# m4rch1n0/vqvae

Hardware: AMD Instinct MI355X
Metric: latents/sec through geodesic kNN+APSP+K-medoids (higher is better)
Workload: dtype f64-exact(u32 fixed point)

## Files before the change

include/geo_hip.h:

```cpp
#ifndef GEO_HIP_H
#define GEO_HIP_H

#include <stddef.h>
#include <stdint.h>

#ifdef __cplusplus
extern "C" {
#endif

#define GEO_OK 0
#define GEO_E_ARG (-1)
#define GEO_E_WORKSPACE (-2)
#define GEO_E_HIP (-3)
#define GEO_E_NOCONV (-4)

int geo_version(void);
const char *geo_last_error(void);

int geo_set_option(const char *name, int32_t value);

size_t geo_sssp_workspace_bytes(int32_t n, int64_t nnz, int32_t n_sources);

int geo_sssp_multi(const int32_t *indptr, const int32_t *indices, const float *weights,
                   int32_t n, int64_t nnz, const int32_t *sources, int32_t n_sources,
// ... 95 lines not shown
size_t geo_jvp_edges_workspace_bytes(const geo_decoder_desc *dec, int64_t n_nodes, int64_t n_edges, int32_t batch_size);
int geo_decoder_jvp_edges(const geo_decoder_desc *dec, const float *z, int64_t n_nodes,
                          const int32_t *src, const int32_t *dst, int64_t n_edges, int32_t batch_size,
                          float *len_out, void *ws, size_t ws_bytes, void *stream);

#define GEO_JVP_FRONT_VALU 0
#define GEO_JVP_FRONT_MFMA 1
#define GEO_JVP_MID_PIPE 0
#define GEO_JVP_MID_PIPE_DEDUP 1
#define GEO_JVP_MID_ALL 2
#define GEO_JVP_MID_ALL_TANGENT 3
#define GEO_JVP_MID_CHUNK 4
#define GEO_JVP_BACK_MFMA 0
#define GEO_JVP_BACK_PER_NODE 1
#define GEO_JVP_BACK_DEDUP 2
#define GEO_JVP_BACK_VALU 3
#define GEO_JVP_PLAN_FRONT(p) ((p) & 3)
#define GEO_JVP_PLAN_DMAX(p) (16 << (((p) >> 2) & 3))
#define GEO_JVP_PLAN_MID(p) (((p) >> 4) & 15)
#define GEO_JVP_PLAN_BACK(p) (((p) >> 8) & 15)
#define GEO_JVP_PER_NODE 0x1000
#define GEO_JVP_NODE_JACOBIAN 0x2000
#define GEO_JVP_DEDUP 0x4000
#define GEO_JVP_PLAN_PASSES(p) ((p) >> 16)
int geo_jvp_plan(const geo_decoder_desc *dec, int64_t n_nodes, int64_t n_edges, int32_t batch_size, int32_t graph_edges,
                 size_t ws_bytes);

int geo_decoder_jvp_pairs(const geo_decoder_desc *dec, const float *z_start, const float *z_end,
                          int64_t n_edges, int32_t batch_size, float *len_out,
                          void *ws, size_t ws_bytes, void *stream);

typedef struct geo_vanilla_decoder_desc {
    int32_t latent_dim;
    int32_t c1, c2;
    int32_t out_channels;
    int32_t out_size;
    const float *At;
    const float *c;
    const float *w2p;
    const float *scale2;
    const float *shift2;
    const float *w3p;
    const float *b3;
} geo_vanilla_decoder_desc;

size_t geo_vanilla_jvp_workspace_bytes(const geo_vanilla_decoder_desc *dec, int64_t n_edges);
// ... 87 lines not shown
```

vqvae_amd/_lib.py:

```python
import ctypes
import os

import torch

_HERE = os.path.dirname(os.path.abspath(__file__))
LIB_PATH = os.path.join(_HERE, "libgeo_hip.so")

c_p = ctypes.c_void_p
i32, i64, sz = ctypes.c_int32, ctypes.c_int64, ctypes.c_size_t


class DecoderDesc(ctypes.Structure):
    _fields_ = ([(n, i32) for n in ("latent_dim", "c0", "c1", "c2", "out_channels", "out_size", "norm",
                                    "bn_train", "groups1", "groups2")]
                + [("eps", ctypes.c_float)]
                + [(n, c_p) for n in ("w_in", "b_in", "w1", "b1", "g1", "be1", "rm1", "rv1",
                                      "w2", "b2", "g2", "be2", "rm2", "rv2", "w3", "b3")]
                + [("update_running", i32), ("momentum", ctypes.c_float)])


class VanillaDecoderDesc(ctypes.Structure):
    _fields_ = ([(n, i32) for n in ("latent_dim", "c1", "c2", "out_channels", "out_size")]
                + [(n, c_p) for n in ("At", "c", "w2p", "scale2", "shift2", "w3p", "b3")])

# ... 65 lines not shown
    "geo_feature_gram": (ctypes.c_int, [c_p, i64, i32, i64, c_p, c_p, c_p, c_p, sz, c_p]),
    "geo_feature_project": (ctypes.c_int, [c_p, i64, i32, i64, c_p, c_p, c_p, i32, c_p, c_p]),
    "geo_vq_workspace_bytes": (sz, [i64, i32, i32]),
    "geo_vq_forward": (ctypes.c_int, [c_p, i32, i32, i32, i32, c_p, c_p, c_p, i32, i32, ctypes.c_double, ctypes.c_double,
                                      ctypes.c_double, c_p, c_p, c_p, c_p, c_p, c_p, c_p, sz, c_p]),
    "geo_vq_backward": (ctypes.c_int, [c_p, c_p, ctypes.c_double, c_p, i32, c_p, i64, c_p, c_p]),
    "geo_vae_elbo_workspace_bytes": (sz, [i64, i64, i64]),
    "geo_vae_elbo_forward": (ctypes.c_int, [c_p, c_p, c_p, c_p, i64, i64, i64, i32, i32, ctypes.c_double, ctypes.c_double,
                                            ctypes.c_double, i32, c_p, c_p, sz, c_p]),
    "geo_vae_elbo_backward": (ctypes.c_int, [c_p, c_p, c_p, c_p, c_p, c_p, i64, i64, i64, i32, i32, ctypes.c_double,
                                             ctypes.c_double, ctypes.c_double, i32, c_p, c_p, c_p, c_p]),
    "geo_batch_assemble": (ctypes.c_int, [c_p, i64, i32, i32, i32, c_p, i32, c_p, c_p, i32, c_p, c_p, c_p, c_p]),
}

EXPORTS = tuple(_SIGNATURES)

JVP_FRONT = ("valu", "mfma")
JVP_MID = ("pipe", "pipe_dedup", "all", "all_tangent", "chunk")
JVP_BACK = ("mfma", "per_node", "dedup", "valu")


def decode_jvp_plan(code: int) -> dict:
    assert code >= 0, code
    return {"front": JVP_FRONT[code & 3], "dmax": 16 << ((code >> 2) & 3), "mid": JVP_MID[(code >> 4) & 15],
            "back": JVP_BACK[(code >> 8) & 15], "per_node": bool(code & 0x1000), "node_jacobian": bool(code & 0x2000),
            "dedup": bool(code & 0x4000), "passes": code >> 16}
_lib = None


class GeoHipError(RuntimeError):
    pass


def load() -> ctypes.CDLL:
    global _lib
    if _lib is None:
        if not os.path.exists(LIB_PATH):
            raise GeoHipError(
                f"{LIB_PATH} is missing: build it with `make -C vqvae_amd/csrc` "
                "(the geodesic-codebook path has no CPU fallback)")
        L = ctypes.CDLL(LIB_PATH)
        for name, (res, args) in _SIGNATURES.items():
            fn = getattr(L, name)
            fn.restype, fn.argtypes = res, args
        _lib = L
    return _lib


def check(status: int, what: str) -> None:
# ... 3 lines not shown
```

vqvae_amd/csrc/common.hip:

```cpp
#include "geo_common.h"

#include <cstdlib>
#include <cstring>

namespace geo {

namespace {
struct OptionName { const char *name, *env; int Options::*field; };
const OptionName kOptionNames[] = {
    {"sssp_sb", "GEO_SSSP_SB", &Options::sssp_sb},
    {"sssp_act", "GEO_SSSP_ACT", &Options::sssp_act},
    {"sssp_sparse_div", "GEO_SSSP_SPARSE_DIV", &Options::sssp_sparse_div},
    {"sssp_map_div", "GEO_SSSP_MAP_DIV", &Options::sssp_map_div},
    {"sssp_group", "GEO_SSSP_GROUP", &Options::sssp_group},
    {"sssp_grouped_cap", "GEO_SSSP_GROUPED_CAP", &Options::sssp_grouped_cap},
    {"sssp_trace", "GEO_SSSP_TRACE", &Options::sssp_trace},
    {"sssp_u32", "GEO_SSSP_U32", &Options::sssp_u32},
    {"sssp_push", "GEO_SSSP_PUSH", &Options::sssp_push},
    {"sssp_order", "GEO_SSSP_ORDER", &Options::sssp_order},
    {"sssp_delta", "GEO_SSSP_DELTA", &Options::sssp_delta},
    {"sssp_push_blocks", "GEO_SSSP_PUSH_BLOCKS", &Options::sssp_push_blocks},
    {"knn_filter", "GEO_KNN_FILTER", &Options::knn_filter},
    {"kpp_grid", "GEO_KPP_GRID", &Options::kpp_grid},
    {"kpp_profile", "GEO_KPP_PROFILE", &Options::kpp_profile},
    {"jvp_mid", "GEO_JVP_MID", &Options::jvp_mid},
    {"jvp_back_valu", "GEO_JVP_BACK_VALU", &Options::jvp_back_valu},
    {"jvp_front_valu", "GEO_JVP_FRONT_VALU", &Options::jvp_front_valu},
    {"jvp_per_node", "GEO_JVP_PER_NODE", &Options::jvp_per_node},
    {"jvp_node_jacobian", "GEO_JVP_NODE_JACOBIAN", &Options::jvp_node_jacobian},
    {"jvp_start_dedup", "GEO_JVP_START_DEDUP", &Options::jvp_start_dedup},
};
Options from_environment() {
    Options o;
    for (const OptionName &e : kOptionNames) {
        const char *v = getenv(e.env);
        if (!v) continue;
        if (e.field == &Options::jvp_mid) o.jvp_mid = v[0] == 'c' ? 2 : (v[0] == 'a' ? 3 : atoi(v));
        else o.*(e.field) = atoi(v);
    }
    return o;
}
}

Options &options() {
    static Options o = from_environment();
    return o;
}

static thread_local char g_err[512] = "";

void set_error(const char *fmt, ...) {
    va_list ap;
    va_start(ap, fmt);
// ... 87 lines not shown
    int rc = scan_rec(sums, offs, t, ar, s);
    if (rc != GEO_OK) return rc;
    scan_add_kernel<<<dim3((unsigned)t), dim3(SCAN_THREADS), 0, s>>>(out, offs, n, t);
    GEO_LAUNCH_CHECK();
    return GEO_OK;
}

int exclusive_scan_i32(const int32_t *in, int32_t *out, int64_t n, void *tmp, size_t tmp_bytes,
                       int64_t *total_host, hipStream_t stream) {
    Arena ar(tmp, tmp_bytes);
    int rc = scan_rec(in, out, n, ar, stream);
    if (rc != GEO_OK) return rc;
    if (total_host) {
        int32_t tot = 0;
        GEO_HIP_CHECK(hipMemcpyAsync(&tot, out + n, sizeof(int32_t), hipMemcpyDeviceToHost, stream));
        GEO_HIP_CHECK(hipStreamSynchronize(stream));
        *total_host = tot;
    }
    return GEO_OK;
}

}

extern "C" int geo_version(void) { return 104; }
extern "C" const char *geo_last_error(void) { return geo::g_err; }

extern "C" int geo_set_option(const char *name, int32_t value) {
    if (name)
        for (const geo::OptionName &e : geo::kOptionNames)
            if (strcmp(name, e.name) == 0) {
                geo::options().*(e.field) = value;
                return GEO_OK;
            }
    geo::set_error("geo_set_option: unknown option '%s'", name ? name : "(null)");
    return GEO_E_ARG;
}
```

vqvae_amd/csrc/geo_common.h:

```cpp
#pragma once
#include <hip/hip_runtime.h>

#include <cstdarg>
#include <cstdint>
#include <cstdio>

#include "geo_hip.h"

namespace geo {

void set_error(const char *fmt, ...);

#define GEO_HIP_CHECK(expr)                                                                      \
    do {                                                                                         \
        hipError_t _e = (expr);                                                                  \
        if (_e != hipSuccess) {                                                                  \
            geo::set_error("%s failed: %s (%s:%d)", #expr, hipGetErrorString(_e), __FILE__, __LINE__); \
            return GEO_E_HIP;                                                                    \
        }                                                                                        \
    } while (0)

#define GEO_REQUIRE(cond, ...)              \
    do {                                    \
        if (!(cond)) {                      \
            geo::set_error(__VA_ARGS__);    \
            return GEO_E_ARG;               \
        }                                   \
    } while (0)

#define GEO_LAUNCH_CHECK() GEO_HIP_CHECK(hipGetLastError())

struct Options {
    int sssp_sb = -1, sssp_act = 1, sssp_sparse_div = -1, sssp_map_div = -1, sssp_group = 1, sssp_grouped_cap = 256,
        sssp_trace = 0, sssp_u32 = 1, sssp_push = 1 ,
        sssp_delta = 8 , sssp_order = 0 , sssp_push_blocks = 64, knn_filter = 1, kpp_grid = 256, kpp_profile = 0, jvp_mid = 0 ,
        jvp_back_valu = 0, jvp_front_valu = 0, jvp_per_node = 1 ,
        jvp_node_jacobian = 1 ,
        jvp_start_dedup = 1 ;
};
Options &options();

static inline size_t align_up(size_t x, size_t a = 256) { return (x + a - 1) / a * a; }

struct Arena {
    char *base;
    size_t size, off;
    Arena(void *p, size_t n) : base(static_cast<char *>(p)), size(n), off(0) {}
    template <typename T>
    T *take(size_t count) {
        size_t bytes = align_up(count * sizeof(T));
        if (off + bytes > size) return nullptr;
        T *r = reinterpret_cast<T *>(base + off);
        off += bytes;
        return r;
    }
};

size_t scan_tmp_bytes(int64_t n);
int exclusive_scan_i32(const int32_t *in, int32_t *out, int64_t n, void *tmp, size_t tmp_bytes,
                       int64_t *total_host, hipStream_t stream);

// ... 9 lines not shown
```

vqvae_amd/csrc/jvp.hip:

```cpp
#include "geo_common.h"

#include <cmath>
#include <cstdlib>
#include <type_traits>
#include <vector>

namespace {

constexpr int TS = 32;
constexpr int NC = 128;
constexpr int MAX_BLOCKS = 4;
constexpr int FRONT_MAX_N1 = 1024;
constexpr int BACK_TS = 8;

typedef float f32x16 __attribute__((ext_vector_type(16)));
typedef __bf16 bf16x8 __attribute__((ext_vector_type(8)));
typedef unsigned short u16x8 __attribute__((ext_vector_type(8)));

struct Shape {
    int d, c0, c1, c2, co, s_out, pad3, p_out;
    int n1, n2;
    int opix_per_chunk, n_chunks;
};

// ... 119 lines not shown
            }
#pragma unroll
            for (int u = 0; u < 2; ++u) {
                const float x = u ? x2.y : x2.x, t = u ? t2.y : t2.x;
                pre[(slot0 + s + u) * n1 + n] = x;
                tpre[(slot0 + s + u) * n1 + n] = t;
                if (valid_s[s + u]) {
                    sx += x; sxx += (double)x * x; st += t; sxt += (double)x * t;
                }
            }
        }
        if (want_stats) { ps[n][0] = sx; ps[n][1] = sxx; ps[n][2] = st; ps[n][3] = sxt; }
    }
    if (want_stats) {
        __syncthreads();
        const int c1 = n1 / 4;
        for (int c = threadIdx.x; c < c1; c += 256) {
            double a0 = 0, a1 = 0, a2 = 0, a3 = 0;
#pragma unroll
            for (int px = 0; px < 4; ++px) { a0 += ps[px * c1 + c][0]; a1 += ps[px * c1 + c][1]; a2 += ps[px * c1 + c][2]; a3 += ps[px * c1 + c][3]; }
            double *p = partial + ((size_t)tile * c1 + c) * 4;
            p[0] = a0; p[1] = a1; p[2] = a2; p[3] = a3;
        }
    }
}

template <int DMAX>
__global__ __launch_bounds__(256) void front_mfma_kernel(const float *__restrict__ z, const int32_t *__restrict__ src,
                                                        const int32_t *__restrict__ dst, const float *__restrict__ z_start,
                                                        const float *__restrict__ z_end, int64_t e_base, int64_t n_edges,
                                                        int batch, int tiles_per_group, int d, int n1,
                                                        const float *__restrict__ M01, const float *__restrict__ b01,
                                                        float *__restrict__ pre, float *__restrict__ tpre,
                                                        double *__restrict__ partial, int want_stats) {
    __shared__ float zp[TS][DMAX + 1];
    __shared__ float dz[TS][DMAX + 1];
    __shared__ int valid_s[TS];
    __shared__ double ps[FRONT_MAX_N1][4];
    const int tile = blockIdx.x;
    const int group = tile / tiles_per_group, tg = tile % tiles_per_group;
    const int chunk = group >> 1, side = group & 1;
    for (int i = threadIdx.x; i < TS * DMAX; i += 256) {
        const int s = i / DMAX, k = i % DMAX;
        const int within = tg * TS + s;
        const int64_t e = e_base + (int64_t)chunk * batch + within;
        float a = 0.f, b = 0.f;
// ... 836 lines not shown
            tile = next;
        }
        epilogue(tile - (int)gridDim.x);
    }
#undef GEO_STAGE_FULL
#undef GEO_PIPE_SEP
#undef GEO_PB
#undef GEO_PIPE_PIXEL
}

__global__ __launch_bounds__(256) void start_runs_kernel(const int32_t *__restrict__ src, int64_t e_base, int64_t n_edges, int batch,
                                                        int slots_per_group, int32_t *__restrict__ row_map, int32_t *__restrict__ rep,
                                                        int32_t *__restrict__ n_compact) {
    __shared__ int wsum[4];
    __shared__ int carry_s;
    const int chunk = blockIdx.x;
    const size_t g0 = (size_t)chunk * 2 * slots_per_group;
    const int lane = threadIdx.x & 63, wave = threadIdx.x >> 6;
    int carry = 0;
    for (int w0 = 0; w0 < slots_per_group; w0 += 256) {
        const int within = w0 + (int)threadIdx.x;
        const int64_t e = e_base + (int64_t)chunk * batch + within;
        const bool valid = within < slots_per_group && within < batch && e < n_edges;
        const bool head = valid && (within == 0 || src[e] != src[e - 1]);
        const unsigned long long m = __ballot(head);
        const int below = __popcll(m & ((1ull << lane) - 1ull));
        if (lane == 0) wsum[wave] = __popcll(m);
        __syncthreads();
        int before = carry, total = carry;
        for (int w = 0; w < 4; ++w) { if (w < wave) before += wsum[w]; total += wsum[w]; }
        const int k = before + below + (head ? 1 : 0) - 1;
        if (within < slots_per_group) {
            row_map[g0 + within] = (int32_t)(g0 + (valid ? k : 0));
            if (head) rep[g0 + k] = (int32_t)(g0 + within);
        }
        carry = total;
        __syncthreads();
    }
    if (threadIdx.x == 0) { carry_s = carry; n_compact[chunk] = carry; }
    __syncthreads();
    const int cnt = carry_s, padded = (cnt + TS - 1) / TS * TS;
    for (int k = cnt + (int)threadIdx.x; k < padded; k += 256) rep[g0 + k] = (int32_t)g0;
}

template <bool TT>
__global__ __launch_bounds__(512, 2) void mid_start_kernel(const float *__restrict__ pre1, const float *__restrict__ tpre1,
                                                          const NormConst *__restrict__ consts1, int tiles_per_group,
                                                          const unsigned short *__restrict__ B3, const float *__restrict__ b2,
                                                          float *__restrict__ pre2, float *__restrict__ tpre2,
                                                          double *__restrict__ partial2, const int32_t *__restrict__ row_map,
                                                          const int32_t *__restrict__ rep, const int32_t *__restrict__ n_compact,
                                                          int64_t e_base, int64_t n_edges, int batch) {
    constexpr int C1 = 128, LDK = C1 + 8, KS = C1 / 16, NL = 4, c2 = 64, n1 = 4 * C1, n2 = 16 * c2;
    typedef float f32x2 __attribute__((ext_vector_type(2)));
    __shared__ __attribute__((aligned(16))) unsigned short A3[2][3][2][TS][LDK];
    const int chunk = blockIdx.y, group = 2 * chunk;
    const int ncomp = TT ? 0 : n_compact[chunk];
    auto run = [&](int item) {
    const int lt0 = 2 * item;
    const bool live1 = TT ? lt0 + 1 < tiles_per_group : (lt0 + 1) * TS < ncomp;
    const int tile0 = group * tiles_per_group + lt0, tile1 = live1 ? tile0 + 1 : tile0;
    const int lane = threadIdx.x & 63, wave = __builtin_amdgcn_readfirstlane((int)(threadIdx.x >> 6));
    const int wq = wave & 3, wg = wave >> 2;
    const int r = lane & 31, h = lane >> 5;
    f32x16 accp[NL], acct[NL];
#pragma unroll
    for (int lc = 0; lc < NL; ++lc)
#pragma unroll
        for (int i = 0; i < 16; ++i) { accp[lc][i] = 0.f; acct[lc][i] = 0.f; }

    const int k0p = 2 * lane, s0p = 4 * wave;
    const NormConst *kp = consts1 + (size_t)group * C1 + k0p;
    const NormConst kA = kp[0], kB = kp[1];
    size_t xrow[2][4];
#pragma unroll
    for (int i = 0; i < 4; ++i) {
        const size_t s0 = (size_t)tile0 * TS + s0p + i, s1 = (size_t)tile1 * TS + s0p + i;
        xrow[0][i] = TT ? s0 : (size_t)__builtin_amdgcn_readfirstlane(rep[s0]);
        xrow[1][i] = TT ? s1 : (size_t)__builtin_amdgcn_readfirstlane(rep[s1]);
    }
    f32x2 rx[2][4], rt[2][4];
    auto fetch = [&](int nx) {
#pragma unroll
        for (int hh = 0; hh < 2; ++hh)
#pragma unroll
            for (int i = 0; i < 4; ++i) {
                const size_t off = xrow[hh][i] * n1 + (size_t)MidGeom::pix(nx) * C1 + k0p;
                rx[hh][i] = *reinterpret_cast<const f32x2 *>(pre1 + off);
                if (TT) rt[hh][i] = *reinterpret_cast<const f32x2 *>(tpre1 + off);
            }
    };
    fetch(0);
    auto stage_px = [&](int buf, int nx) {
#pragma unroll
        for (int hh = 0; hh < 2; ++hh)
#pragma unroll
            for (int i = 0; i < 4; ++i) {
                float a0, t0, a1, t1;
                norm_relu(kA, rx[hh][i].x, TT ? rt[hh][i].x : 0.f, &a0, &t0);
                norm_relu(kB, rx[hh][i].y, TT ? rt[hh][i].y : 0.f, &a1, &t1);
                unsigned w[3];
                if (TT) split3_pair(t0, t1, w[0], w[1], w[2]);
                else split3_pair(a0, a1, w[0], w[1], w[2]);
#pragma unroll
                for (int part = 0; part < 3; ++part) *reinterpret_cast<unsigned *>(&A3[buf][part][hh][s0p + i][k0p]) = w[part];
            }
        if (nx < 4) {
            fetch(nx);
            __builtin_amdgcn_sched_group_barrier(0x020, TT ? 16 : 8, 0);
// ... 495 lines not shown
    b += geo::align_up((size_t)16 * s.c2 * 192 * 3 * 2);
    b += 2 * geo::align_up(slots * s.n1 * 4) + 2 * geo::align_up(slots * s.n2 * 4);
    b += geo::align_up(tiles * s.n1 * 4 * 8) + geo::align_up(tiles * s.n2 * 4 * 8);
    b += geo::align_up((groups + 1) * s.c1 * sizeof(NormConst)) + geo::align_up((groups + 1) * s.c2 * sizeof(NormConst));
    b += geo::align_up((groups + 1) * (size_t)(s.c1 > s.c2 ? s.c1 : s.c2) * sizeof(float2));
    b += geo::align_up(slots * 4) * 2;
    if (dc->norm == 2) b += 2 * geo::align_up(slots * 32 * sizeof(float4));
    p->bytes = b + 4096;
    return true;
}

enum { BACK_NODE_PRIMAL = 15 };

struct Route {
    int status = GEO_OK;
    char error[192] = "";
    Plan pl = {};
    int64_t run_edges = 0, passes = 0;
    bool batch_stats = false, track = false, group_norm = false;
    int front = GEO_JVP_FRONT_VALU, dmax = 16;
    int mid = GEO_JVP_MID_CHUNK, back = GEO_JVP_BACK_VALU;
    int back_nt = 0;
    int parts2 = 16;
    bool per_node = false, node_jacobian = false, dedup = false;
    size_t back_lds = 0;
    size_t jac_np = 0, jac_extra_bytes = 0;
    size_t bytes = 0;
};

bool route_error(Route *r, int status, const char *fmt, ...) {
    va_list ap;
    va_start(ap, fmt);
    vsnprintf(r->error, sizeof(r->error), fmt, ap);
    va_end(ap);
    r->status = status;
    return false;
}

bool make_route(const geo_decoder_desc *dc, const geo::Options &o, bool graph_edges, int64_t n_nodes, int64_t n_edges, int batch,
                const size_t *ws_bytes, Route *r) {
    *r = Route{};
    if (!dc) return route_error(r, GEO_E_ARG, "geo_decoder_jvp: null pointer");
    if (batch <= 0) return route_error(r, GEO_E_ARG, "geo_decoder_jvp: batch_size must be positive");
    Plan base;
    if (n_edges < 0 || n_nodes < 0 || !make_plan(dc, n_edges, batch, &base))
        return route_error(r, GEO_E_ARG, "geo_decoder_jvp: unsupported decoder (out_size %d, c2=%d must divide %d)", dc->out_size,
                           dc->c2, NC);
// ... 15 lines not shown
    Plan jpl;
    const int64_t n_pseudo = (n_nodes + 1) / 2 * s.d;
    size_t jac_bytes = 0;
    if (per_node_kernels && n_nodes > 0 && n_edges > 0 && s.d <= 16 && o.jvp_node_jacobian != 0 &&
        (o.jvp_node_jacobian != 1 || 4 * n_edges >= 3 * n_nodes * s.d) && n_pseudo < (int64_t)1 << 31 &&
        make_plan(dc, n_pseudo, batch, &jpl) && node_slots <= jpl.pass_slots()) {
        r->jac_np = (size_t)r->back_nt * 32;
        r->jac_extra_bytes = 2 * geo::align_up((size_t)n_pseudo * 4) + geo::align_up((size_t)n_nodes * s.d * r->jac_np * 4);
        jac_bytes = r->jac_extra_bytes + jpl.bytes + node_bytes(s, n_nodes);
    }
    r->bytes = jac_bytes > per_edge_end_bytes ? jac_bytes : per_edge_end_bytes;
    const size_t ws = ws_bytes ? *ws_bytes : r->bytes;
    r->node_jacobian = jac_bytes && ws >= jac_bytes;
    r->pl = r->node_jacobian ? jpl : base;
    r->run_edges = r->node_jacobian ? n_pseudo : n_edges;
    const int64_t chunks = (r->run_edges + batch - 1) / batch;
    r->passes = (chunks + r->pl.chunks_per_pass - 1) / r->pl.chunks_per_pass;
    const size_t run_ws = ws - (r->node_jacobian ? r->jac_extra_bytes : 0);
    r->per_node = per_node_kernels && node_slots && node_slots <= r->pl.pass_slots() &&
                  run_ws >= r->pl.bytes + node_bytes(s, n_nodes);
    const size_t slots = r->pl.pass_slots(), tiles = slots / TS, groups = (size_t)r->pl.chunks_per_pass * 2;
    r->dedup = r->batch_stats && graph_edges && mid_pipe && back_mfma && o.jvp_start_dedup != 0 &&
               (2 * slots + groups) * 4 <= tiles * s.n1 * 4 * 8 && (size_t)r->back_nt * 32 <= (size_t)s.n1;

    r->mid = r->per_node ? GEO_JVP_MID_ALL_TANGENT
           : mid_pipe    ? (r->dedup ? GEO_JVP_MID_PIPE_DEDUP : GEO_JVP_MID_PIPE)
           : mid_all     ? GEO_JVP_MID_ALL
                         : GEO_JVP_MID_CHUNK;
    r->parts2 = mid_pipe && !r->per_node ? 4 : (mid_all ? 1 : 16);
    r->back = r->dedup ? GEO_JVP_BACK_DEDUP : r->per_node ? GEO_JVP_BACK_PER_NODE : back_mfma ? GEO_JVP_BACK_MFMA : GEO_JVP_BACK_VALU;
    r->back_lds = ((size_t)2 * BACK_TS * 16 * (s.c2 + 4) + (size_t)16 * s.co * (s.c2 + 4) + (size_t)BACK_TS * s.p_out) * 4;

    if (!(s.d >= 1 && s.d <= 64)) return route_error(r, GEO_E_ARG, "geo_decoder_jvp: latent_dim %d not in [1,64]", s.d);
    if (!(s.c1 == 128 || s.c1 == 64 || s.c1 == 32))
        return route_error(r, GEO_E_ARG, "geo_decoder_jvp: dec_channels[1]=%d not in {32,64,128}", s.c1);
    if (!(dc->norm >= 0 && dc->norm <= 2)) return route_error(r, GEO_E_ARG, "geo_decoder_jvp: unknown norm code %d", dc->norm);
    if (s.c2 % 16 != 0) return route_error(r, GEO_E_ARG, "geo_decoder_jvp: dec_channels[2]=%d must be a multiple of 16", s.c2);
    if (r->back_lds > 160 * 1024)
        return route_error(r, GEO_E_ARG, "geo_decoder_jvp: decoder too wide for the back kernel (%zu B LDS)", r->back_lds);
    if (run_ws < r->pl.bytes) return route_error(r, GEO_E_WORKSPACE, "geo_decoder_jvp: workspace %zu < %zu", run_ws, r->pl.bytes);
    if (r->group_norm && !(dc->groups1 == 32 && dc->groups2 == 32 && s.c2 == 64 && back_mfma && mid_all))
        return route_error(r, GEO_E_ARG,
                           "geo_decoder_jvp: GroupNorm needs 32 groups per layer and dec_channels[2] == 64 (got %d/%d groups, c2=%d)",
                           dc->groups1, dc->groups2, s.c2);
    return true;
}

int encode_route(const Route &r) {
    const int64_t passes = r.passes < 0x7fff ? r.passes : 0x7fff;
    return r.front | (r.dmax == 16 ? 0 : (r.dmax == 32 ? 1 : 2)) << 2 | r.mid << 4 | r.back << 8 |
           (r.per_node ? GEO_JVP_PER_NODE : 0) | (r.node_jacobian ? GEO_JVP_NODE_JACOBIAN : 0) | (r.dedup ? GEO_JVP_DEDUP : 0) |
           (int)passes << 16;
}

struct Buffers {
    float *M01, *b01, *B2p, *W3p, *pre1, *tpre1, *pre2, *tpre2, *norms;
    unsigned short *B3, *W3b;
    double *part1, *part2; NormConst *k1, *k2;
    float2 *stats;
    int32_t *slot_valid;
    float4 *gs1, *gs2;
    float *pre2_node, *sg_node;
    int32_t *row_map, *rep, *n_compact;
    float *sg_compact, *jac;
    ChunkTable tab;
};

struct Pass {
    int mid, back;
    int64_t tiles, e_base, n_edges;
    int tiles_per_group, batch, unit_d, stat;
    const float *z, *z_start, *z_end;
    const int32_t *src, *dst;
    float *mid_pre2;
    const float *back_pre2;
    int64_t slots() const { return tiles * TS; }
    int64_t groups() const { return tiles / tiles_per_group; }
};

template <int... Vs, class F>
void pick_int(int v, F &&f) { ((v == Vs ? (void)f(std::integral_constant<int, Vs>{}) : (void)0), ...); }
template <class F>
void pick_bool(bool v, F &&f) { if (v) f(std::true_type{}); else f(std::false_type{}); }

int cu_count(int *n) {
    static int n_cu = 0;
    if (n_cu == 0) {
        int devid = 0, cus = 0;
        GEO_HIP_CHECK(hipGetDevice(&devid));
        GEO_HIP_CHECK(hipDeviceGetAttribute(&cus, hipDeviceAttributeMultiprocessorCount, devid));
        n_cu = cus > 0 ? cus : 256;
    }
    *n = n_cu;
    return GEO_OK;
}

int launch_front(const Route &r, const Pass &p, const Buffers &b, hipStream_t stream) {
    const Shape &s = r.pl.sh;
    if (r.front == GEO_JVP_FRONT_MFMA)
        pick_int<32, 64>(r.dmax, [&](auto dm) {
            front_mfma_kernel<decltype(dm)::value><<<(unsigned)p.tiles, 256, 0, stream>>>(
                p.z, p.src, p.dst, p.z_start, p.z_end, p.e_base, p.n_edges, p.batch, p.tiles_per_group, s.d, s.n1, b.M01, b.b01,
                b.pre1, b.tpre1, b.part1, p.stat);
        });
    else
        pick_int<16, 32, 64>(r.dmax, [&](auto dm) {
            front_kernel<decltype(dm)::value><<<(unsigned)p.tiles, 256, 0, stream>>>(
                p.z, p.src, p.dst, p.z_start, p.z_end, p.e_base, p.n_edges, p.batch, p.tiles_per_group, s.d, s.n1, b.M01, b.b01,
                b.pre1, b.tpre1, b.part1, p.stat, p.unit_d);
        });
    GEO_LAUNCH_CHECK();
    return GEO_OK;
}

int launch_stats(const Route &r, const geo_decoder_desc *dc, int layer, const Pass &p, const Buffers &b, hipStream_t stream) {
    const Shape &s = r.pl.sh;
    const bool l1 = layer == 1;
    const int C = l1 ? s.c1 : s.c2, npx = l1 ? 4 : 16;
    if (p.stat) {
        finalize_batch_kernel<<<geo::grid_for(p.groups() * C, 256), 256, 0, stream>>>(
            l1 ? b.part1 : b.part2, p.tiles_per_group, l1 ? 1 : r.parts2, npx, C, p.e_base, p.n_edges, p.batch, l1 ? dc->g1 : dc->g2,
            l1 ? dc->be1 : dc->be2, dc->eps, l1 ? b.k1 : b.k2, (int)p.groups(), r.track ? b.stats : nullptr);
// ... 2 lines not shown
                b.stats, (int)p.groups(), C, dc->momentum, const_cast<float *>(l1 ? dc->rm1 : dc->rm2),
                const_cast<float *>(l1 ? dc->rv1 : dc->rv2));
        GEO_LAUNCH_CHECK();
    }
    if (r.group_norm) {
        const int32_t *prim_row = nullptr;
        if (!l1 && p.back == GEO_JVP_BACK_PER_NODE) {
            slot_node_kernel<<<geo::grid_for(p.slots(), 256), 256, 0, stream>>>(p.src, p.dst, p.e_base, p.n_edges, p.batch,
                                                                                p.tiles_per_group, p.slots(), b.slot_valid);
            prim_row = b.slot_valid;
        }
        group_stats_kernel<<<geo::grid_for(p.slots() * 32, 256), 256, 0, stream>>>(
            l1 ? b.pre1 : p.back_pre2, l1 ? b.tpre1 : b.tpre2, p.slots(), npx, C, 32, dc->eps, l1 ? b.gs1 : b.gs2, prim_row);
        GEO_LAUNCH_CHECK();
    }
    return GEO_OK;
}

int launch_mid(const Route &r, const geo_decoder_desc *dc, const Pass &p, const Buffers &b, hipStream_t stream) {
    const Shape &s = r.pl.sh;
    if (p.mid == GEO_JVP_MID_PIPE || p.mid == GEO_JVP_MID_PIPE_DEDUP) {
        const bool dedup = p.mid == GEO_JVP_MID_PIPE_DEDUP;
        const int64_t chunks = p.groups() / 2;
        if (dedup) {
            start_runs_kernel<<<(unsigned)chunks, 256, 0, stream>>>(p.src, p.e_base, p.n_edges, p.batch, p.tiles_per_group * TS,
                                                                    b.row_map, b.rep, b.n_compact);
            GEO_LAUNCH_CHECK();
        }
        int n_cu = 0;
        if (const int rc = cu_count(&n_cu)) return rc;
        const int64_t pipe_tiles = dedup ? p.tiles / 2 : p.tiles;
        const unsigned grid = (unsigned)std::min<int64_t>(pipe_tiles, n_cu);
        pick_bool(dedup, [&](auto end_only) {
            mid_pipe_kernel<decltype(end_only)::value><<<grid, 512, 0, stream>>>(
                b.pre1, b.tpre1, b.k1, p.stat, p.tiles_per_group, (int)pipe_tiles, s.c2, b.B3, dc->b2, p.mid_pre2, b.tpre2, b.part2,
                p.stat, p.e_base, p.n_edges, p.batch);
        });
        GEO_LAUNCH_CHECK();
        if (dedup) {
            mid_start_kernel<false><<<dim3(1, (unsigned)chunks), 512, 0, stream>>>(
                b.pre1, b.tpre1, b.k1, p.tiles_per_group, b.B3, dc->b2, p.mid_pre2, b.tpre2, b.part2, b.row_map, b.rep, b.n_compact,
                p.e_base, p.n_edges, p.batch);
            GEO_LAUNCH_CHECK();
            mid_start_kernel<true><<<dim3((unsigned)((p.tiles_per_group + 1) / 2), (unsigned)chunks), 512, 0, stream>>>(
                b.pre1, b.tpre1, b.k1, p.tiles_per_group, b.B3, dc->b2, p.mid_pre2, b.tpre2, b.part2, b.row_map, b.rep, b.n_compact,
                p.e_base, p.n_edges, p.batch);
            GEO_LAUNCH_CHECK();
        }
    } else if (p.mid == GEO_JVP_MID_ALL || p.mid == GEO_JVP_MID_ALL_TANGENT) {
        pick_int<128, 64, 32>(s.c1, [&](auto c1) {
            pick_bool(r.group_norm, [&](auto gn) {
                pick_bool(p.mid == GEO_JVP_MID_ALL_TANGENT, [&](auto tangent_only) {
                    mid_all_kernel<decltype(c1)::value, decltype(gn)::value, decltype(tangent_only)::value>
                        <<<(unsigned)p.tiles, 512, 0, stream>>>(b.pre1, b.tpre1, b.k1, p.stat, p.tiles_per_group, s.c2, b.B3, dc->b2,
                                                                p.mid_pre2, b.tpre2, b.part2, p.stat, b.slot_valid, b.gs1, p.e_base,
                                                                p.n_edges, p.batch);
                });
            });
        });
        GEO_LAUNCH_CHECK();
    } else {
        pick_int<128, 64, 32>(s.c1, [&](auto c1) {
            mid_bf16_kernel<decltype(c1)::value><<<dim3((unsigned)p.tiles, (unsigned)s.n_chunks), 256, 0, stream>>>(
                b.pre1, b.tpre1, b.k1, p.stat, p.tiles_per_group, b.tab, s.opix_per_chunk, s.c2, b.B3, dc->b2, p.mid_pre2, b.tpre2,
                b.part2, p.stat, b.slot_valid);
        });
        GEO_LAUNCH_CHECK();
    }
    return GEO_OK;
// ... 21 lines not shown
                p.back_pre2, b.tpre2, b.k2, 1, p.tiles_per_group, s.co, s.s_out, b.W3b, dc->b3, b.norms, nullptr, b.sg_compact, nullptr,
                nullptr, 0, 0, 1, nullptr, 0, b.row_map, nullptr, 1);
            return;
        }
        pick_bool(r.group_norm, [&](auto gn) {
            constexpr bool GN = decltype(gn)::value;
            if (p.back == GEO_JVP_BACK_MFMA)
                back_mfma_kernel<NT, GN, 0><<<tiles, 256, 0, stream>>>(p.back_pre2, b.tpre2, b.k2, p.stat, p.tiles_per_group, s.co,
                                                                      s.s_out, b.W3b, dc->b3, b.norms, b.gs2);
            else if (p.back == GEO_JVP_BACK_PER_NODE)
                back_mfma_kernel<NT, GN, 1><<<tiles, 256, 0, stream>>>(p.back_pre2, b.tpre2, b.k2, 0, p.tiles_per_group, s.co, s.s_out,
                                                                      b.W3b, dc->b3, b.norms, b.gs2, b.sg_node, p.src, p.dst, p.e_base,
                                                                      p.n_edges, p.batch, b.jac, p.unit_d);
            else
                back_mfma_kernel<NT, GN, 2><<<tiles, 256, 0, stream>>>(p.back_pre2, b.tpre2, b.k2, 0, p.tiles_per_group, s.co, s.s_out,
                                                                      b.W3b, dc->b3, b.norms, b.gs2, b.sg_node);
        });
    });
    GEO_LAUNCH_CHECK();
    return GEO_OK;
}

int launch_pass(const Route &r, const geo_decoder_desc *dc, const Pass &p, const Buffers &b, hipStream_t stream) {
    if (const int rc = launch_front(r, p, b, stream)) return rc;
    if (const int rc = launch_stats(r, dc, 1, p, b, stream)) return rc;
    if (const int rc = launch_mid(r, dc, p, b, stream)) return rc;
    if (const int rc = launch_stats(r, dc, 2, p, b, stream)) return rc;
    return launch_back(r, dc, p, b, stream);
}

int run_jvp(const geo_decoder_desc *dc, const Route &r, const float *z, int64_t n_nodes, const int32_t *src, const int32_t *dst,
            const float *z_start, const float *z_end, int64_t n_edges, float *len_out, void *ws, size_t ws_bytes,
            hipStream_t stream) {
    const Plan &pl = r.pl;
    const Shape &s = pl.sh;
    const int batch = pl.batch;
    const size_t slots = pl.pass_slots(), tiles = slots / TS, groups = (size_t)pl.chunks_per_pass * 2;

    geo::Arena ar(ws, ws_bytes);
    Buffers b = {};
    int32_t *psrc = nullptr, *pdst = nullptr;
    if (r.node_jacobian) {
        psrc = ar.take<int32_t>((size_t)r.run_edges);
        pdst = ar.take<int32_t>((size_t)r.run_edges);
        b.jac = ar.take<float>((size_t)n_nodes * s.d * r.jac_np);
        GEO_REQUIRE(b.jac != nullptr, "geo_decoder_jvp_edges: workspace carve failed");
    }
    b.M01 = ar.take<float>((size_t)s.d * s.n1);
    b.b01 = ar.take<float>((size_t)s.n1);
    b.B2p = ar.take<float>((size_t)s.n_chunks * MAX_BLOCKS * s.c1 * NC);
    b.B3 = ar.take<unsigned short>((size_t)s.n_chunks * MAX_BLOCKS * s.c1 * NC * 3);
    b.W3p = ar.take<float>((size_t)16 * s.co * s.c2);
    b.W3b = ar.take<unsigned short>((size_t)16 * s.c2 * 192 * 3);
    b.pre1 = ar.take<float>(slots * s.n1); b.tpre1 = ar.take<float>(slots * s.n1);
    b.pre2 = ar.take<float>(slots * s.n2); b.tpre2 = ar.take<float>(slots * s.n2);
    b.part1 = ar.take<double>(tiles * s.n1 * 4); b.part2 = ar.take<double>(tiles * s.n2 * 4);
    b.k1 = ar.take<NormConst>((groups + 1) * s.c1); b.k2 = ar.take<NormConst>((groups + 1) * s.c2);
    b.norms = ar.take<float>(slots);
    b.stats = ar.take<float2>((groups + 1) * (size_t)(s.c1 > s.c2 ? s.c1 : s.c2));
    b.slot_valid = ar.take<int32_t>(slots);
    if (r.group_norm) { b.gs1 = ar.take<float4>(slots * 32); b.gs2 = ar.take<float4>(slots * 32); }
    const size_t node_slots = round_up_to_tile(n_nodes);
    if (r.per_node) {
        b.pre2_node = ar.take<float>(node_slots * s.n2);
        b.sg_node = ar.take<float>(node_slots * (size_t)((s.p_out + 31) / 32) * 32);
    }
    GEO_REQUIRE(b.slot_valid && (!r.group_norm || b.gs2) && (!r.per_node || b.sg_node), "geo_decoder_jvp: workspace carve failed");
    if (r.dedup) {
        b.row_map = reinterpret_cast<int32_t *>(b.part1); b.rep = b.row_map + slots; b.n_compact = b.rep + slots;
        b.sg_compact = b.pre1;
    }

    make_chunks(s, &b.tab);
    int bad_chunk = 0;
    GEO_REQUIRE(!(s.n_chunks == 8 && s.opix_per_chunk == 2) || chunks_match_mid_geom(b.tab, &bad_chunk),
                "geo_decoder_jvp: chunk table / MidGeom mismatch (chunk %d)", bad_chunk);
    compose_front_kernel<<<geo::grid_for((int64_t)(s.d + 1) * s.n1, 256), 256, 0, stream>>>(
        dc->w_in, dc->b_in, dc->w1, dc->b1, s.d, s.c0, s.c1, b.M01, b.b01);
    GEO_LAUNCH_CHECK();
    pack_mid_kernel<<<geo::grid_for((int64_t)s.n_chunks * MAX_BLOCKS * s.c1 * NC, 256), 256, 0, stream>>>(
        dc->w2, s.c1, s.c2, b.tab, s.n_chunks, s.opix_per_chunk, b.B2p);
    GEO_LAUNCH_CHECK();
    pack_back_kernel<<<geo::grid_for(16 * s.co * s.c2, 256), 256, 0, stream>>>(dc->w3, s.c2, s.co, b.W3p);
    GEO_LAUNCH_CHECK();
    if (r.back != GEO_JVP_BACK_VALU) {
        pack_back_bf16_kernel<<<geo::grid_for((int64_t)16 * s.c2 * r.back_nt * 32, 256), 256, 0, stream>>>(
            dc->w3, s.c2, s.co, s.s_out, s.pad3, r.back_nt * 32, b.W3b);
        GEO_LAUNCH_CHECK();
    }
    pack_mid_bf16_kernel<<<geo::grid_for((int64_t)s.n_chunks * MAX_BLOCKS * s.c1 * NC, 256), 256, 0, stream>>>(
        b.B2p, s.c1, s.n_chunks, b.B3);
    GEO_LAUNCH_CHECK();
// ... 117 lines not shown
```

Measured before the change: 2.309 million.

## Compute start and end front activations in one edge kernel with shared tangent

Adds a front_edge_kernel that loads each edge's src and dst latents once and computes the start pre-activation, end pre-activation and tangent together. Start rows are written only at run heads, and batch statistics for both sides are accumulated in the same pass. The mid start kernel then reads deduplicated start rows through buffer loads indexed via row_map/rep, and start_runs is moved ahead of the front stage. The aim is to avoid separate front passes and redundant start-row work. In exchange it adds layout coupling: row_map is offset inside part1, and the path only applies when n1 equals 512.

```diff
diff --git a/include/geo_hip.h b/include/geo_hip.h
--- a/include/geo_hip.h
+++ b/include/geo_hip.h
@@ -141,6 +141,7 @@
 #define GEO_JVP_PER_NODE 0x1000
 #define GEO_JVP_NODE_JACOBIAN 0x2000
 #define GEO_JVP_DEDUP 0x4000
+#define GEO_JVP_FRONT_ONCE 0x8000
 #define GEO_JVP_PLAN_PASSES(p) ((p) >> 16)
 int geo_jvp_plan(const geo_decoder_desc *dec, int64_t n_nodes, int64_t n_edges, int32_t batch_size, int32_t graph_edges,
                  size_t ws_bytes);
diff --git a/vqvae_amd/_lib.py b/vqvae_amd/_lib.py
--- a/vqvae_amd/_lib.py
+++ b/vqvae_amd/_lib.py
@@ -111,9 +111,14 @@
 
 def decode_jvp_plan(code: int) -> dict:
     assert code >= 0, code
-    return {"front": JVP_FRONT[code & 3], "dmax": 16 << ((code >> 2) & 3), "mid": JVP_MID[(code >> 4) & 15],
-            "back": JVP_BACK[(code >> 8) & 15], "per_node": bool(code & 0x1000), "node_jacobian": bool(code & 0x2000),
-            "dedup": bool(code & 0x4000), "passes": code >> 16}
+    r = {"front": JVP_FRONT[code & 3], "dmax": 16 << ((code >> 2) & 3), "mid": JVP_MID[(code >> 4) & 15],
+         "back": JVP_BACK[(code >> 8) & 15], "per_node": bool(code & 0x1000), "node_jacobian": bool(code & 0x2000),
+         "dedup": bool(code & 0x4000), "passes": code >> 16}
+    if code & 0x8000:
+        r["front_once"] = True
+    return r
+
+
 _lib = None
 
 
diff --git a/vqvae_amd/csrc/common.hip b/vqvae_amd/csrc/common.hip
--- a/vqvae_amd/csrc/common.hip
+++ b/vqvae_amd/csrc/common.hip
@@ -29,6 +29,7 @@
     {"jvp_per_node", "GEO_JVP_PER_NODE", &Options::jvp_per_node},
     {"jvp_node_jacobian", "GEO_JVP_NODE_JACOBIAN", &Options::jvp_node_jacobian},
     {"jvp_start_dedup", "GEO_JVP_START_DEDUP", &Options::jvp_start_dedup},
+    {"jvp_front_once", "GEO_JVP_FRONT_ONCE", &Options::jvp_front_once},
 };
 Options from_environment() {
     Options o;
@@ -162,7 +163,7 @@
 
 }
 
-extern "C" int geo_version(void) { return 104; }
+extern "C" int geo_version(void) { return 105; }
 extern "C" const char *geo_last_error(void) { return geo::g_err; }
 
 extern "C" int geo_set_option(const char *name, int32_t value) {
diff --git a/vqvae_amd/csrc/geo_common.h b/vqvae_amd/csrc/geo_common.h
--- a/vqvae_amd/csrc/geo_common.h
+++ b/vqvae_amd/csrc/geo_common.h
@@ -36,7 +36,8 @@
         sssp_delta = 8 , sssp_order = 0 , sssp_push_blocks = 64, knn_filter = 1, kpp_grid = 256, kpp_profile = 0, jvp_mid = 0 ,
         jvp_back_valu = 0, jvp_front_valu = 0, jvp_per_node = 1 ,
         jvp_node_jacobian = 1 ,
-        jvp_start_dedup = 1 ;
+        jvp_start_dedup = 1 ,
+        jvp_front_once = 1 ;
 };
 Options &options();
 
diff --git a/vqvae_amd/csrc/jvp.hip b/vqvae_amd/csrc/jvp.hip
--- a/vqvae_amd/csrc/jvp.hip
+++ b/vqvae_amd/csrc/jvp.hip
@@ -165,6 +165,120 @@
             double *p = partial + ((size_t)tile * c1 + c) * 4;
             p[0] = a0; p[1] = a1; p[2] = a2; p[3] = a3;
         }
+    }
+}
+
+__device__ __forceinline__ bool start_run_head(const int32_t *__restrict__ src, int64_t e, int within) {
+    return within == 0 || src[e] != src[e - 1];
+}
+
+constexpr int FRONT_EDGE_N1 = 512;
+template <int DMAX>
+__global__ __launch_bounds__(256) void front_edge_kernel(const float *__restrict__ z, const int32_t *__restrict__ src,
+                                                        const int32_t *__restrict__ dst, int64_t e_base, int64_t n_edges,
+                                                        int batch, int tiles_per_group, int d, const float *__restrict__ M01,
+                                                        const float *__restrict__ b01, float *__restrict__ pre,
+                                                        float *__restrict__ tpre, double *__restrict__ partial) {
+    constexpr int N1 = FRONT_EDGE_N1, C1 = N1 / 4;
+    constexpr int NCOL = DMAX == 16 ? 2 : 1;
+    __shared__ __attribute__((aligned(8))) float za[DMAX][TS];
+    __shared__ __attribute__((aligned(8))) float zb[DMAX][TS];
+    __shared__ __attribute__((aligned(8))) float dz[DMAX][TS];
+    typedef float f32x2 __attribute__((ext_vector_type(2)));
+    __shared__ int valid_s[TS], head_s[TS];
+    __shared__ double ps[2][N1][4];
+    const int chunk = blockIdx.x / tiles_per_group, tg = blockIdx.x % tiles_per_group;
+    const size_t tile_s = (size_t)(2 * chunk) * tiles_per_group + tg, tile_e = tile_s + tiles_per_group;
+    for (int i = threadIdx.x; i < TS * d; i += 256) {
+        const int s = i / d, k = i % d;
+        const int within = tg * TS + s;
+        const int64_t e = e_base + (int64_t)chunk * batch + within;
+        float a = 0.f, b = 0.f;
+        const bool ok = within < batch && e < n_edges;
+        if (ok) {
+            a = z[(int64_t)src[e] * d + k];
+            b = z[(int64_t)dst[e] * d + k];
+        }
+        za[k][s] = a;
+        zb[k][s] = b;
+        dz[k][s] = b - a;
+        if (k == 0) {
+            valid_s[s] = ok ? 1 : 0;
+            head_s[s] = ok && start_run_head(src, e, within) ? 1 : 0;
+        }
+    }
+    for (int i = threadIdx.x; i < TS * (DMAX - d); i += 256) {
+        const int s = i / (DMAX - d), k = d + i % (DMAX - d);
+        za[k][s] = 0.f;
+        zb[k][s] = 0.f;
+        dz[k][s] = 0.f;
+    }
+    __syncthreads();
+    float *__restrict__ pre_s = pre + tile_s * TS * N1;
+    float *__restrict__ pre_e = pre + tile_e * TS * N1;
+    float *__restrict__ tpre_e = tpre + tile_e * TS * N1;
+    for (int n0 = threadIdx.x; n0 < N1; n0 += 256 * NCOL) {
+        float m[NCOL][DMAX], bias[NCOL];
+#pragma unroll
+        for (int c = 0; c < NCOL; ++c) {
+#pragma unroll
+            for (int k = 0; k < DMAX; ++k) m[c][k] = k < d ? M01[(size_t)k * N1 + n0 + 256 * c] : 0.f;
+            bias[c] = b01[n0 + 256 * c];
+        }
+        double se[NCOL][4], ss[NCOL][4];
+#pragma unroll
+        for (int c = 0; c < NCOL; ++c)
+#pragma unroll
+            for (int j = 0; j < 4; ++j) { se[c][j] = 0; ss[c][j] = 0; }
+        for (int s = 0; s < TS; s += 2) {
+            f32x2 xe[NCOL], xs[NCOL], t2[NCOL];
+#pragma unroll
+            for (int c = 0; c < NCOL; ++c) { xe[c] = {bias[c], bias[c]}; xs[c] = {bias[c], bias[c]}; t2[c] = {0.f, 0.f}; }
+#pragma unroll
+            for (int k = 0; k < DMAX; ++k) {
+                const f32x2 a2 = *reinterpret_cast<const f32x2 *>(&za[k][s]);
+                const f32x2 b2 = *reinterpret_cast<const f32x2 *>(&zb[k][s]);
+                const f32x2 d2 = *reinterpret_cast<const f32x2 *>(&dz[k][s]);
+#pragma unroll
+                for (int c = 0; c < NCOL; ++c) {
+                    const f32x2 mk = {m[c][k], m[c][k]};
+                    xe[c] = __builtin_elementwise_fma(b2, mk, xe[c]);
+                    xs[c] = __builtin_elementwise_fma(a2, mk, xs[c]);
+                    t2[c] = __builtin_elementwise_fma(d2, mk, t2[c]);
+                }
+            }
+#pragma unroll
+            for (int u = 0; u < 2; ++u) {
+                const bool valid = valid_s[s + u] != 0, head = head_s[s + u] != 0;
+#pragma unroll
+                for (int c = 0; c < NCOL; ++c) {
+                    const size_t o = (size_t)(s + u) * N1 + n0 + 256 * c;
+                    const float x = u ? xe[c].y : xe[c].x, y = u ? xs[c].y : xs[c].x, t = u ? t2[c].y : t2[c].x;
+                    pre_e[o] = x;
+                    tpre_e[o] = t;
+                    if (head) pre_s[o] = y;
+                    if (valid) {
+                        se[c][0] += x; se[c][1] += (double)x * x; se[c][2] += t; se[c][3] += (double)x * t;
+                        ss[c][0] += y; ss[c][1] += (double)y * y; ss[c][2] += t; ss[c][3] += (double)y * t;
+                    }
+                }
+            }
+        }
+#pragma unroll
+        for (int c = 0; c < NCOL; ++c)
+#pragma unroll
+            for (int j = 0; j < 4; ++j) { ps[0][n0 + 256 * c][j] = ss[c][j]; ps[1][n0 + 256 * c][j] = se[c][j]; }
+    }
+    __syncthreads();
+    {
+        const int side = threadIdx.x / C1, c = threadIdx.x % C1;
+        double a0 = 0, a1 = 0, a2 = 0, a3 = 0;
+#pragma unroll
+        for (int px = 0; px < 4; ++px) {
+            a0 += ps[side][px * C1 + c][0]; a1 += ps[side][px * C1 + c][1]; a2 += ps[side][px * C1 + c][2]; a3 += ps[side][px * C1 + c][3];
+        }
+        double *p = partial + ((side ? tile_e : tile_s) * C1 + c) * 4;
+        p[0] = a0; p[1] = a1; p[2] = a2; p[3] = a3;
     }
 }
 
@@ -1047,7 +1161,7 @@
         const int within = w0 + (int)threadIdx.x;
         const int64_t e = e_base + (int64_t)chunk * batch + within;
         const bool valid = within < slots_per_group && within < batch && e < n_edges;
-        const bool head = valid && (within == 0 || src[e] != src[e - 1]);
+        const bool head = valid && start_run_head(src, e, within);
         const unsigned long long m = __ballot(head);
         const int below = __popcll(m & ((1ull << lane) - 1ull));
         if (lane == 0) wsum[wave] = __popcll(m);
@@ -1068,7 +1182,7 @@
     for (int k = cnt + (int)threadIdx.x; k < padded; k += 256) rep[g0 + k] = (int32_t)g0;
 }
 
-template <bool TT>
+template <bool TT, bool ONCE = false>
 __global__ __launch_bounds__(512, 2) void mid_start_kernel(const float *__restrict__ pre1, const float *__restrict__ tpre1,
                                                           const NormConst *__restrict__ consts1, int tiles_per_group,
                                                           const unsigned short *__restrict__ B3, const float *__restrict__ b2,
@@ -1097,19 +1211,41 @@
     const int k0p = 2 * lane, s0p = 4 * wave;
     const NormConst *kp = consts1 + (size_t)group * C1 + k0p;
     const NormConst kA = kp[0], kB = kp[1];
+    static_assert(TT || !ONCE, "ONCE selects where the tangent launch reads");
     size_t xrow[2][4];
+    const size_t g0 = (size_t)group * tiles_per_group * TS, group_slots = (size_t)tiles_per_group * TS;
+    unsigned xoff[2][4], toff[2];
+    __amdgpu_buffer_rsrc_t x_src, t_src;
 #pragma unroll
     for (int i = 0; i < 4; ++i) {
         const size_t s0 = (size_t)tile0 * TS + s0p + i, s1 = (size_t)tile1 * TS + s0p + i;
-        xrow[0][i] = TT ? s0 : (size_t)__builtin_amdgcn_readfirstlane(rep[s0]);
-        xrow[1][i] = TT ? s1 : (size_t)__builtin_amdgcn_readfirstlane(rep[s1]);
-    }
+        if (ONCE) {
+            xoff[0][i] = (unsigned)(__builtin_amdgcn_readfirstlane(rep[__builtin_amdgcn_readfirstlane(row_map[s0])]) - (int)g0) * (n1 * 4u);
+            xoff[1][i] = (unsigned)(__builtin_amdgcn_readfirstlane(rep[__builtin_amdgcn_readfirstlane(row_map[s1])]) - (int)g0) * (n1 * 4u);
+        } else {
+            xrow[0][i] = TT ? s0 : (size_t)__builtin_amdgcn_readfirstlane(rep[s0]);
+            xrow[1][i] = TT ? s1 : (size_t)__builtin_amdgcn_readfirstlane(rep[s1]);
+        }
+    }
+    if (ONCE) {
+        x_src = __builtin_amdgcn_make_buffer_rsrc(const_cast<float *>(pre1 + g0 * n1), 0, (int)(group_slots * n1 * 4), 0x00020000);
+        t_src = __builtin_amdgcn_make_buffer_rsrc(const_cast<float *>(tpre1 + (g0 + group_slots) * n1), 0, (int)(group_slots * n1 * 4), 0x00020000);
+        toff[0] = (unsigned)(lt0 * TS + s0p) * (n1 * 4u);
+        toff[1] = (unsigned)((live1 ? lt0 + 1 : lt0) * TS + s0p) * (n1 * 4u);
+    }
+    const unsigned v_pair = (unsigned)k0p * 4u;
     f32x2 rx[2][4], rt[2][4];
     auto fetch = [&](int nx) {
 #pragma unroll
         for (int hh = 0; hh < 2; ++hh)
 #pragma unroll
             for (int i = 0; i < 4; ++i) {
+                if (ONCE) {
+                    const int px_off = MidGeom::pix(nx) * C1 * 4;
+                    rx[hh][i] = __builtin_bit_cast(f32x2, __builtin_amdgcn_raw_buffer_load_b64(x_src, v_pair, xoff[hh][i] + px_off, 0));
+                    rt[hh][i] = __builtin_bit_cast(f32x2, __builtin_amdgcn_raw_buffer_load_b64(t_src, v_pair, toff[hh] + i * n1 * 4 + px_off, 0));
+                    continue;
+                }
                 const size_t off = xrow[hh][i] * n1 + (size_t)MidGeom::pix(nx) * C1 + k0p;
                 rx[hh][i] = *reinterpret_cast<const f32x2 *>(pre1 + off);
                 if (TT) rt[hh][i] = *reinterpret_cast<const f32x2 *>(tpre1 + off);
@@ -1651,7 +1787,7 @@
     int mid = GEO_JVP_MID_CHUNK, back = GEO_JVP_BACK_VALU;
     int back_nt = 0;
     int parts2 = 16;
-    bool per_node = false, node_jacobian = false, dedup = false;
+    bool per_node = false, node_jacobian = false, dedup = false, front_once = false;
     size_t back_lds = 0;
     size_t jac_np = 0, jac_extra_bytes = 0;
     size_t bytes = 0;
@@ -1713,6 +1849,9 @@
     const size_t slots = r->pl.pass_slots(), tiles = slots / TS, groups = (size_t)r->pl.chunks_per_pass * 2;
     r->dedup = r->batch_stats && graph_edges && mid_pipe && back_mfma && o.jvp_start_dedup != 0 &&
                (2 * slots + groups) * 4 <= tiles * s.n1 * 4 * 8 && (size_t)r->back_nt * 32 <= (size_t)s.n1;
+    r->front_once = r->dedup && r->front == GEO_JVP_FRONT_VALU && o.jvp_front_once != 0 && s.n1 == FRONT_EDGE_N1 &&
+                    tiles * s.c1 * 4 * 8 + (2 * slots + groups) * 4 <= tiles * s.n1 * 4 * 8 &&
+                    (size_t)base.slots_per_group * s.n1 * 4 < ((size_t)1 << 31);
 
     r->mid = r->per_node ? GEO_JVP_MID_ALL_TANGENT
            : mid_pipe    ? (r->dedup ? GEO_JVP_MID_PIPE_DEDUP : GEO_JVP_MID_PIPE)
@@ -1741,7 +1880,7 @@
     const int64_t passes = r.passes < 0x7fff ? r.passes : 0x7fff;
     return r.front | (r.dmax == 16 ? 0 : (r.dmax == 32 ? 1 : 2)) << 2 | r.mid << 4 | r.back << 8 |
            (r.per_node ? GEO_JVP_PER_NODE : 0) | (r.node_jacobian ? GEO_JVP_NODE_JACOBIAN : 0) | (r.dedup ? GEO_JVP_DEDUP : 0) |
-           (int)passes << 16;
+           (r.front_once ? GEO_JVP_FRONT_ONCE : 0) | (int)passes << 16;
 }
 
 struct Buffers {
@@ -1786,9 +1925,21 @@
     return GEO_OK;
 }
 
+int launch_start_runs(const Pass &p, const Buffers &b, hipStream_t stream) {
+    start_runs_kernel<<<(unsigned)(p.groups() / 2), 256, 0, stream>>>(p.src, p.e_base, p.n_edges, p.batch, p.tiles_per_group * TS,
+                                                                     b.row_map, b.rep, b.n_compact);
+    GEO_LAUNCH_CHECK();
+    return GEO_OK;
+}
+
 int launch_front(const Route &r, const Pass &p, const Buffers &b, hipStream_t stream) {
     const Shape &s = r.pl.sh;
-    if (r.front == GEO_JVP_FRONT_MFMA)
+    if (r.front_once)
+        pick_int<16, 32, 64>(r.dmax, [&](auto dm) {
+            front_edge_kernel<decltype(dm)::value><<<(unsigned)(p.tiles / 2), 256, 0, stream>>>(
+                p.z, p.src, p.dst, p.e_base, p.n_edges, p.batch, p.tiles_per_group, s.d, b.M01, b.b01, b.pre1, b.tpre1, b.part1);
+        });
+    else if (r.front == GEO_JVP_FRONT_MFMA)
         pick_int<32, 64>(r.dmax, [&](auto dm) {
             front_mfma_kernel<decltype(dm)::value><<<(unsigned)p.tiles, 256, 0, stream>>>(
                 p.z, p.src, p.dst, p.z_start, p.z_end, p.e_base, p.n_edges, p.batch, p.tiles_per_group, s.d, s.n1, b.M01, b.b01,
@@ -1837,11 +1988,8 @@
     if (p.mid == GEO_JVP_MID_PIPE || p.mid == GEO_JVP_MID_PIPE_DEDUP) {
         const bool dedup = p.mid == GEO_JVP_MID_PIPE_DEDUP;
         const int64_t chunks = p.groups() / 2;
-        if (dedup) {
-            start_runs_kernel<<<(unsigned)chunks, 256, 0, stream>>>(p.src, p.e_base, p.n_edges, p.batch, p.tiles_per_group * TS,
-                                                                    b.row_map, b.rep, b.n_compact);
-            GEO_LAUNCH_CHECK();
-        }
+        if (dedup && !r.front_once)
+            if (const int rc = launch_start_runs(p, b, stream)) return rc;
         int n_cu = 0;
         if (const int rc = cu_count(&n_cu)) return rc;
         const int64_t pipe_tiles = dedup ? p.tiles / 2 : p.tiles;
@@ -1857,9 +2005,12 @@
                 b.pre1, b.tpre1, b.k1, p.tiles_per_group, b.B3, dc->b2, p.mid_pre2, b.tpre2, b.part2, b.row_map, b.rep, b.n_compact,
                 p.e_base, p.n_edges, p.batch);
             GEO_LAUNCH_CHECK();
-            mid_start_kernel<true><<<dim3((unsigned)((p.tiles_per_group + 1) / 2), (unsigned)chunks), 512, 0, stream>>>(
-                b.pre1, b.tpre1, b.k1, p.tiles_per_group, b.B3, dc->b2, p.mid_pre2, b.tpre2, b.part2, b.row_map, b.rep, b.n_compact,
-                p.e_base, p.n_edges, p.batch);
+            pick_bool(r.front_once, [&](auto once) {
+                mid_start_kernel<true, decltype(once)::value>
+                    <<<dim3((unsigned)((p.tiles_per_group + 1) / 2), (unsigned)chunks), 512, 0, stream>>>(
+                        b.pre1, b.tpre1, b.k1, p.tiles_per_group, b.B3, dc->b2, p.mid_pre2, b.tpre2, b.part2, b.row_map, b.rep,
+                        b.n_compact, p.e_base, p.n_edges, p.batch);
+            });
             GEO_LAUNCH_CHECK();
         }
     } else if (p.mid == GEO_JVP_MID_ALL || p.mid == GEO_JVP_MID_ALL_TANGENT) {
@@ -1927,6 +2078,8 @@
 }
 
 int launch_pass(const Route &r, const geo_decoder_desc *dc, const Pass &p, const Buffers &b, hipStream_t stream) {
+    if (r.front_once)
+        if (const int rc = launch_start_runs(p, b, stream)) return rc;
     if (const int rc = launch_front(r, p, b, stream)) return rc;
     if (const int rc = launch_stats(r, dc, 1, p, b, stream)) return rc;
     if (const int rc = launch_mid(r, dc, p, b, stream)) return rc;
@@ -1972,7 +2125,7 @@
     }
     GEO_REQUIRE(b.slot_valid && (!r.group_norm || b.gs2) && (!r.per_node || b.sg_node), "geo_decoder_jvp: workspace carve failed");
     if (r.dedup) {
-        b.row_map = reinterpret_cast<int32_t *>(b.part1); b.rep = b.row_map + slots; b.n_compact = b.rep + slots;
+        b.row_map = reinterpret_cast<int32_t *>(b.part1 + (r.front_once ? tiles * s.c1 * 4 : 0)); b.rep = b.row_map + slots; b.n_compact = b.rep + slots;
         b.sg_compact = b.pre1;
     }
 
```

New measurement: 2.416 million (median of 6 runs). +4.6%, better.
